# MIT-SPARK/Kimera-Semantics

Hardware: AMD Instinct MI355X
Metric: Mvoxel-updates/s + frames/s, 640×480 @5cm voxels, 1/2/4/8 MI355X (higher is better)
Workload: dtype f32; 1 GPU; bag-replay stand-in: 640x480 depth+label trajectory (room), 'fast' integrator, 5 cm voxels, 5 m rays, trunc 0.2 m, p=0.8; pipeline_frames=12, parallelism=frame-sharded x1, points_per_frame=305657, rays_per_frame=85307, updates_per_frame=502687

## Files before the change

kimera_semantics_amd/csrc/ks_hip.hip:

```cpp

#include <atomic>
#include <chrono>
#include <condition_variable>
#include <mutex>
#include <thread>
#include <cstring>
#include <string.h>

#include <dlfcn.h>
#include <hip/hip_runtime.h>
#include <hip/hip_ext.h>
#include <rccl/rccl.h>

#include <algorithm>
#include <iterator>
#include <cmath>
#include <cstdio>
#include <cstring>
#include <string>
#include <unordered_map>
#include <vector>

#include "../../include/ks_hip.h"
#include "ks_device_math.h"
// ... 880 lines not shown
                       (const uint32_t*)vres, c->d_eo_plain);
  return KS_OK;
}

int ensure_exact_slots(ks_ctx* c, size_t cap_marks, size_t cap_x) {
  if (!c->eo_device) return KS_OK;
  int rc;
  const int n_slots = c->cfg.pipeline_frames ? c->n_slots : 1;
  for (int i = 0; i < n_slots; ++i) {
    FrameSlot& S = c->slot[i];
    if (!S.d_eo_ctl) {
      if ((rc = S.d_eo_ctl.alloc(c, 1))) return rc;
      if ((rc = S.d_eo_tab.alloc(c, (size_t)1 << kSetBits))) return rc;
      HIPCHK(c, hipMemsetAsync(S.d_eo_tab, 0, sizeof(uint4) << kSetBits, c->stream));
      if ((rc = S.eo_committed.create(c, hipEventDisableTiming))) return rc;
    }
    if (S.eo_cap_marks < cap_marks) {
      S.eo_cap_marks = 0;
      for (int b = 0; b < 2; ++b) {
        if ((rc = S.d_eo_keys[b].alloc(c, cap_marks))) return rc;
        if ((rc = S.d_eo_vals[b].alloc(c, cap_marks))) return rc;
      }
      if ((rc = S.d_eo_sort_ws.alloc(c, ksrs::ws_words_dev(cap_marks, 3)))) return rc;
      if ((rc = S.d_eo_hitb.alloc(c, cap_marks))) return rc;
      if ((rc = S.d_eo_hseq.alloc(c, cap_marks))) return rc;
      if ((rc = S.d_eo_where.alloc(c, cap_marks))) return rc;
      if ((rc = S.d_eo_bits_a.alloc(c, cap_marks / 64 + 2))) return rc;
      if ((rc = S.d_eo_bits_b.alloc(c, cap_marks / 64 + 2))) return rc;
      S.eo_cap_marks = cap_marks;
    }
    if ((rc = S.d_eo_xnode.reserve(c, 2 * cap_x, 2 * cap_x))) return rc;
  }
  c->eo_cap_marks = cap_marks;
  c->eo_cap_x = cap_x;
  ++c->buffers_epoch;
  HIPCHK(c, hipStreamSynchronize(c->stream));
  return KS_OK;
}
int ensure_exact_points(ks_ctx* c, size_t cap) {
  if (!c->eo_device) return KS_OK;
  int rc;
  for (int i = 0; i < (c->cfg.pipeline_frames ? c->n_slots : 1); ++i) {
    FrameSlot& S = c->slot[i];
    for (DevBuf<uint32_t>* p : {&S.d_eo_cnt_b, &S.d_eo_ux, &S.d_eo_dirty, &S.d_eo_list[0], &S.d_eo_list[1], &S.d_eo_chg, &S.d_eo_consulted, &S.d_eo_lp})
      if ((rc = p->alloc(c, cap))) return rc;
    if ((rc = S.d_eo_bt.alloc(c, cap / kScanBlock + 2))) return rc;
// ... 78 lines not shown
    hipLaunchKernelGGL(k_eo2_scan, dim3(nb4k, nb), dim3(1024), 0, st, Bt);
    hipLaunchKernelGGL(k_eo2_emit<8>, dim3((uint32_t)((n + 31) / 32), nb), dim3(256), lds, st, Bt);
    HIPCHK(c, ksrs::sort_dev_batch<uint64_t>(Rs, (int)nb, S0.d_eo_sort_ws.size(), S0.eo_cap_marks, 44, 64, st));
    hipLaunchKernelGGL(k_eo2_bits, dim3(gm, nb), dim3(256), 0, st, Bt, 0u);
    hipLaunchKernelGGL(k_eo2_where, dim3(gm, nb), dim3(256), 0, st, Bt);
    enqueue_sweeps(c, Bt, nb, c->eo_sweeps, st);
    return KS_OK;
  } else {
    hipLaunchKernelGGL(k_eo2_scan, dim3(nb4k, nb), dim3(1024), 0, st, Bt);
    hipLaunchKernelGGL(k_eo2_emit<64>, dim3((uint32_t)((n + 255) / 256), nb), dim3(256), lds, st, Bt);
    HIPCHK(c, ksrs::sort_dev_batch<uint64_t>(Rs, (int)nb, S0.d_eo_sort_ws.size(), S0.eo_cap_marks, 44, 64, st));
    hipLaunchKernelGGL(k_eo2_hits, dim3(gm, nb), dim3(256), 0, st, Bt);
    hipLaunchKernelGGL(k_eo2_stop0, dim3(gn, nb), dim3(256), 0, st, Bt);
    hipLaunchKernelGGL(k_eo2_bits, dim3(gm, nb), dim3(256), 0, st, Bt, 1u);
  }
  const uint32_t gr = (uint32_t)std::min<size_t>((n + 3) / 4, 2048);
  for (int r = 1; r <= c->eo_bulk_rounds; ++r) {
    const uint32_t g = S0.wide ? gr : std::min(gr, r == 1 ? 2048u : r == 2 ? 1024u : r <= 4 ? 512u : 256u);
    hipLaunchKernelGGL(k_eo2_eval, dim3(g, nb), dim3(256), 0, st, Bt, (uint32_t)r);
    hipLaunchKernelGGL(k_eo2_propagate, dim3(g, nb), dim3(256), 0, st, Bt, (uint32_t)r);
  }
  return KS_OK;
}
void enqueue_exact_finish(ks_ctx* c, FrameSlot& S, hipStream_t st) {
  const EoView E = eo_view(c, S);
  hipLaunchKernelGGL(k_eo2_finish, dim3(1), dim3(kEoFinishThreads), 0, st, E, (uint32_t)c->eo_bulk_rounds + 1u, 1u);
  hipLaunchKernelGGL(k_eo2_commit, dim3(1024), dim3(256), 0, st, E);
}

template <typename Enqueue> hipGraphExec_t capture_graph(hipStream_t sm, Enqueue enqueue) {
  hipGraph_t g = nullptr;
  hipGraphExec_t out = nullptr;
  bool ok = hipStreamBeginCapture(sm, hipStreamCaptureModeRelaxed) == hipSuccess;
  if (ok) {
    const int rc = enqueue();
    ok = hipStreamEndCapture(sm, &g) == hipSuccess && g != nullptr && rc == KS_OK;
  }
  if (ok) ok = hipGraphInstantiate(&out, g, nullptr, nullptr, 0) == hipSuccess;
  if (g) (void)hipGraphDestroy(g);
  return ok ? out : nullptr;
}
struct BatchLaunch {
  ks_ctx* c;
  FrameSlot* const* slots;
  uint32_t nb;
  FrameSlot& S0;
  hipStream_t sm;
  const BatchView& V;
  size_t steps_max;
  uint64_t key;
// ... 3 lines not shown
    for (uint32_t k = 0; k < nb; ++k) Bt.v[k] = eo_view(c, *slots[k]);
    for (int chunk = 1;; ++chunk) {
      bool going = false;
      for (uint32_t k = 0; k < nb; ++k) {
        uint32_t w[2] = {0u, 0u};
        HIPCHK(c, hipMemcpyAsync(&w[0], &slots[k]->d_eo_ctl->sw_prev, sizeof(uint32_t), hipMemcpyDeviceToHost, sm));
        HIPCHK(c, hipMemcpyAsync(&w[1], &slots[k]->d_eo_ctl->fail, sizeof(uint32_t), hipMemcpyDeviceToHost, sm));
        HIPCHK(c, hipStreamSynchronize(sm));
        going = going || (w[0] != 0u && w[1] == 0u);
      }
      if (!going || chunk >= c->eo_sweep_chunks) break;
      enqueue_sweeps(c, Bt, nb, c->eo_sweeps, sm);
    }
    hipLaunchKernelGGL(k_eo2_sweep_done, dim3(nb), dim3(64), 0, sm, Bt);
    return KS_OK;
  }
  int exact_device() const {
    int rc;
    auto seed_and_rounds = [&] {
      enqueue_stage_b(c, V, nb, S0.wide, sm, steps_max, 1);
      return enqueue_exact_rounds(c, slots, nb, sm);
    };
    auto finish = [&] {
      for (uint32_t k = 0; k < nb; ++k) enqueue_exact_finish(c, *slots[k], sm);
      return KS_OK;
    };
    auto emission = [&] { return enqueue_stage_b(c, V, nb, S0.wide, sm, steps_max, 2), KS_OK; };
    bool graphs = c->use_graphs && !S0.wide;
    if (graphs && (G.key != key || !G.g1 || !G.g2 || !G.g3)) {
      std::lock_guard<std::mutex> cap(c->capture_mu);
      G.reset();
      if ((G.g1 = capture_graph(sm, seed_and_rounds)) && (G.g2 = capture_graph(sm, finish)) && (G.g3 = capture_graph(sm, emission))) {
        G.key = key;
      } else {
        (void)hipGetLastError();
        G.reset();
        c->use_graphs = graphs = false;
      }
    }
    if (graphs) HIPCHK(c, hipGraphLaunch(G.g1, sm));
    else if ((rc = seed_and_rounds()) || (S0.wide && (rc = sweeps_host_driven()))) return rc;
    if (c->eo_last_commit && c->eo_last_commit != S0.eo_committed) HIPCHK(c, hipStreamWaitEvent(sm, c->eo_last_commit, 0));
    if (graphs) HIPCHK(c, hipGraphLaunch(G.g2, sm));
    else finish();
    HIPCHK(c, hipEventRecord(S0.eo_committed, sm));
    c->eo_last_commit = S0.eo_committed;
    if (graphs) HIPCHK(c, hipGraphLaunch(G.g3, sm));
// ... 103 lines not shown
  F.clear_bit = (cfg.method == KS_METHOD_MERGED) ? (1u << pb) : 0u;
  F.seq_bits = pb + (cfg.method == KS_METHOD_MERGED ? 1u : 0u);
  F.inv_order = F.sorted_order ? c->d_inv_order : nullptr;
  std::memcpy(F.dynamic_labels, cfg.dynamic_labels, 32);
  F.early_out = c->uses_early_out;
}
void begin_prof_set(ks_ctx* c, FrameSlot& S, size_t n) {
  const int set = (int)(c->frame_no % kProfSets);
  resolve_prof(c, set);
  ProfSet& P = c->pset[set];
  P.used = true;
  P.complete = P.applied = false;
  P.stages = c->profiling == 1;
  P.apply = c->profiling == 1 || (c->frame_no % 4) == 0;
  P.n_points = n;
  P.n_pairs = 0;
  S.prof_set = set;
}
int stage_a_fast(ks_ctx* c, FrameSlot& S, const float* d_xyz, const uint8_t* d_rgba, const uint8_t* d_labels, size_t n) {
  const FrameParams& F = S.F;
  hipStream_t st = c->stream;
  const uint32_t nb1k = (uint32_t)((n + 1023) / 1024);
  hipLaunchKernelGGL(k_points_fast, dim3(nb1k), dim3(1024), 0, st, F, d_xyz, d_rgba, d_labels, c->d_color_lut,
                     S.d_rays, c->d_hash, c->d_skeys32, c->d_pvals, S.d_cnt, S.d_live, S.d_counters);
  stage_mark(c, S.prof_set, 1);
  uint32_t *sk = nullptr, *sv = nullptr;
  if (int rc = sort_pairs(c, c->d_skeys32.get(), c->d_skeys32b.get(), c->d_pvals.get(), c->d_pvals2.get(), n, kSetBits + 1, &sk, &sv)) return rc;
  stage_mark(c, S.prof_set, 2);
  hipLaunchKernelGGL(k_dedup, dim3(nb1k), dim3(1024), 0, st, F, sk, sv, c->d_hash, c->d_start_set, S.d_ray_list, S.d_rays, S.d_cnt, S.d_live, S.d_counters);
  if (c->uses_early_out && n > 0) {
    const uint32_t n_gen = (uint32_t)((n + F.chains - 1) / F.chains);
    uint32_t n_ph = 0;
    while (n_ph < c->seed_phases.size() && c->seed_phases[n_ph].g0 < n_gen) ++n_ph;
    HIPCHK(c, hipMemsetAsync(S.d_seed_n, 0, c->seed_phases.size() * sizeof(uint32_t), st));
    hipLaunchKernelGGL(k_seed_list, dim3((F.chains + 63u) / 64u, n_ph), dim3(64 * kSeedSegs), 0, st, F, (const SeedPhase*)c->d_seed_phases,
                       (const uint8_t*)S.d_live, S.d_seed_gen, S.d_seed_items, S.d_seed_n, S.d_counters);
  }
  hipLaunchKernelGGL(k_dedup_commit, dim3(nb1k), dim3(1024), 0, st, F, sk, sv, c->d_hash, c->d_start_set, S.d_counters);
  return KS_OK;
}
void enqueue_bundle_order(ks_ctx* c, hipStream_t st, size_t n, const uint64_t* sk, const uint32_t* sv) {
  const uint32_t capb = (uint32_t)((c->cap_points + kBoBlock - 1) / kBoBlock);
  const size_t lds_f = (2 * c->cap_points / kBoBlock + 3) * sizeof(uint32_t), lds_e = ((size_t)capb + 2) * sizeof(uint32_t);
  hipLaunchKernelGGL(k_bo_scan_flags, dim3((uint32_t)((2 * n + kBoBlock - 1) / kBoBlock)), dim3(kBoBlock), 0, st, (uint32_t)n, c->bo);
  hipLaunchKernelGGL(k_bo_init, dim3((uint32_t)((n + kBoBlock - 1) / kBoBlock)), dim3(kBoBlock), lds_f, st, (uint32_t)n, sk, sv, c->bo);
  const uint32_t nbb = (uint32_t)((n + kBoBlock - 1) / kBoBlock);
  int e_small = 0;
  while (e_small < c->bo_epochs && c->bo_sched.b[e_small] <= kBoSmallBuckets) ++e_small;
  if (e_small > 0) hipLaunchKernelGGL(k_bo_small, dim3(2), dim3(kBoBlock), 0, st, c->bo, e_small);
  const size_t nh_floor = c->bo_hint_fixed ? (e_small > 0 ? (size_t)c->bo_sched.t[e_small - 1] + 1 : 1) : 2 * (size_t)kBoSmallBuckets;
  const size_t nh = std::min<size_t>(n, std::max<size_t>(c->bo_hint.load(std::memory_order_relaxed), nh_floor));
  int e_last = -1;
  for (int e = e_small; e <= c->bo_epochs; ++e) {
    if (e > 0 && c->bo_sched.t[e - 1] >= nh) break;
    hipLaunchKernelGGL(k_bo_link, dim3(nbb, 2), dim3(kBoBlock), lds_e, st, c->bo, e, (e == e_small && e_small > 0) ? 1 : 0);
    if (e < c->bo_epochs && c->bo_sched.t[e] < nh)
      hipLaunchKernelGGL(k_bo_walk, dim3(nbb, 2), dim3(kBoBlock), 0, st, c->bo, e);
// ... 2330 lines not shown
}

int ks_debug_radix_sort_batch(ks_ctx* c, uint64_t* keys, uint32_t* vals, const uint64_t* counts, int nb, size_t cap, unsigned begin_bit,
                              unsigned end_bit) {
  if (!c || !keys || !vals || !counts || nb < 1 || nb > ksrs::kRsBatch || cap == 0 || cap > 0xffffffffull || begin_bit >= end_bit || end_bit > 64)
    return KS_ERR_INVALID_ARG;
  const int passes = (int)((end_bit - begin_bit + 7) / 8);
  const size_t ws_words = ksrs::ws_words_dev(cap, passes);
  DevBuf<uint64_t> ka[ksrs::kRsBatch], kb[ksrs::kRsBatch];
  DevBuf<uint32_t> va[ksrs::kRsBatch], vb[ksrs::kRsBatch], ws[ksrs::kRsBatch];
  DevBuf<unsigned long long> d_counts;
  int rc;
  if ((rc = d_counts.alloc(c, (size_t)nb))) return rc;
  static_assert(sizeof(unsigned long long) == sizeof(uint64_t), "counts are copied as they are");
  HIPCHK(c, hipMemcpy(d_counts, counts, (size_t)nb * sizeof(uint64_t), hipMemcpyHostToDevice));
  ksrs::DevBatch<uint64_t> B{};
  for (int y = 0; y < nb; ++y) {
    if ((rc = ka[y].alloc(c, cap)) || (rc = kb[y].alloc(c, cap)) || (rc = va[y].alloc(c, cap)) || (rc = vb[y].alloc(c, cap)) || (rc = ws[y].alloc(c, ws_words)))
      return rc;
    HIPCHK(c, hipMemcpy(ka[y], keys + (size_t)y * cap, cap * sizeof(uint64_t), hipMemcpyHostToDevice));
    HIPCHK(c, hipMemcpy(va[y], vals + (size_t)y * cap, cap * sizeof(uint32_t), hipMemcpyHostToDevice));
    HIPCHK(c, hipMemsetAsync(kb[y], 0xA5, cap * sizeof(uint64_t), c->stream));
    HIPCHK(c, hipMemsetAsync(vb[y], 0xA5, cap * sizeof(uint32_t), c->stream));
    B.keys_a[y] = ka[y];
    B.keys_b[y] = kb[y];
    B.vals_a[y] = va[y];
    B.vals_b[y] = vb[y];
    B.n_dev[y] = d_counts.get() + y;
    B.ws[y] = ws[y];
  }
  const hipError_t e = ksrs::sort_dev_batch<uint64_t>(B, nb, ws_words, cap, begin_bit, end_bit, c->stream);
  if (e == hipErrorInvalidValue) return KS_ERR_INVALID_ARG;
  HIPCHK(c, e);
  HIPCHK(c, hipStreamSynchronize(c->stream));
  const bool in_b = (passes & 1) != 0;
  for (int y = 0; y < nb; ++y) {
    HIPCHK(c, hipMemcpy(keys + (size_t)y * cap, in_b ? kb[y].get() : ka[y].get(), cap * sizeof(uint64_t), hipMemcpyDeviceToHost));
    HIPCHK(c, hipMemcpy(vals + (size_t)y * cap, in_b ? vb[y].get() : va[y].get(), cap * sizeof(uint32_t), hipMemcpyDeviceToHost));
  }
  return KS_OK;
}

int ks_get_tile_keys(ks_ctx* c, uint64_t* out, size_t cap, size_t* n) {
  if (!c || !n) return KS_ERR_INVALID_ARG;
  if (int rc = quiesce(c)) return rc;
  HIPCHK(c, hipStreamSynchronize(c->stream));
// ... 1049 lines not shown
```

kimera_semantics_amd/csrc/ks_k_exact.h:

```cpp
#pragma once
#include "ks_k_march.h"

namespace ksk {

struct EoState {
  unsigned long long n_marks;
  unsigned long long n_marks_next;
  uint32_t changed;
  uint32_t pad[3];
};

struct EoBuf {
  const uint64_t* keys;
  const uint32_t* vals;
  uint2* range;
  uint64_t* plain;
};
constexpr uint64_t kEoLow44 = (1ull << 44) - 1ull;

__device__ __forceinline__ uint32_t eo_visited(uint32_t cv) { return (cv & ~kCntBroke) + ((cv & kCntBroke) ? 1u : 0u); }

__global__ void __launch_bounds__(256) k_eo_total(const FrameParams* __restrict__ Fp, const uint32_t* __restrict__ cnt,
                                                  EoState* __restrict__ st) {
  const uint32_t n = Fp->n;
// ... 983 lines not shown
  const EoView& E = Bt.v[blockIdx.y];
  EoCtl* ctl = E.ctl;
  if (ctl->fail) return;
  const uint32_t n = ctl->n_in[round];
  const uint32_t* list = E.list[round & 1u];
  const uint32_t wave = threadIdx.x >> 6, w0 = blockIdx.x * 4u + wave, nw = gridDim.x * 4u;
  if (w0 >= n) return;
  const FrameParams F = *E.F;
  for (uint32_t i = w0; i < n; i += nw) eo2_eval_ray(E, F, list[i], s_w[wave], &ctl->n_chg[round]);
}
__global__ void __launch_bounds__(256) k_eo2_propagate(EoBatch Bt, uint32_t round) {
  __shared__ EoWaveLds s_w[4];
  const EoView& E = Bt.v[blockIdx.y];
  EoCtl* ctl = E.ctl;
  if (ctl->fail) return;
  const uint32_t n = ctl->n_chg[round];
  const uint32_t wave = threadIdx.x >> 6, w0 = blockIdx.x * 4u + wave, nw = gridDim.x * 4u;
  if (blockIdx.x == 0 && threadIdx.x == 0 && n) ctl->rounds = round + 1u;
  if (w0 >= n) return;
  const FrameParams F = *E.F;
  for (uint32_t i = w0; i < n; i += nw) eo2_propagate_ray(E, F, E.chg[i], s_w[wave], E.list[(round + 1u) & 1u], &ctl->n_in[round + 1u]);
}

constexpr uint32_t kEoFinishThreads = 1024;
__global__ void __launch_bounds__(kEoFinishThreads) k_eo2_finish(EoView E, uint32_t first_round, uint32_t chained) {
  __shared__ EoWaveLds s_w[kEoFinishThreads / 64];
  __shared__ uint32_t s_n, s_stop;
  EoCtl* ctl = E.ctl;
  const uint32_t wave = threadIdx.x >> 6, nw = kEoFinishThreads / 64;
  const FrameParams F = *E.F;
  uint32_t cur = first_round & 1u;
  if (threadIdx.x == 0) {
    if (chained && eo2_ld(E.committed) != F.eo_frame) atomicOr(&ctl->fail, kEoFailChain);
    ctl->fin_in[cur] = ctl->n_in[first_round];
    ctl->fin_in[cur ^ 1u] = 0u;
    ctl->fin_chg = 0u;
    s_stop = ctl->fail;
  }
  __syncthreads();
  if (s_stop) {
    if (threadIdx.x == 0) atomicOr(&E.C->err, kErrExact);
    return;
  }
  if (chained) {
    __shared__ uint32_t s_redo;
    if (threadIdx.x == 0) {
      const unsigned long long actual = E.plain[(uint32_t)(F.observed_offset & kSetMask)];
      s_redo = actual != ctl->assumed0 ? 1u : 0u;
      ctl->assumed0 = actual;
    }
    __syncthreads();
    if (s_redo) {
      const uint32_t nc = eo2_ld(&ctl->n_consulted);
      for (uint32_t i = threadIdx.x; i < nc; i += kEoFinishThreads) eo2_mark_dirty(E, eo2_ld(&E.consulted[i]), 0u, E.list[cur], &ctl->fin_in[cur]);
    }
    __syncthreads();
  }
  for (uint32_t it = 0;; ++it) {
    if (threadIdx.x == 0) {
      s_n = eo2_ld(&ctl->fin_in[cur]);
      s_stop = eo2_ld(&ctl->fail) | ((it >= kEoFinishRounds || s_n > kEoFinishRays) ? kEoFailRounds : 0u);
      if (s_n && !s_stop) ctl->rounds += 1u;
    }
    __syncthreads();
    const uint32_t n = s_n;
    if (n == 0u || s_stop) break;
    for (uint32_t i = wave; i < n; i += nw) eo2_eval_ray(E, F, eo2_ld(&E.list[cur][i]), s_w[wave], &ctl->fin_chg);
    __syncthreads();
    if (threadIdx.x == 0) {
      s_n = eo2_ld(&ctl->fin_chg);
      ctl->fin_in[cur] = 0u;
    }
    __syncthreads();
    const uint32_t nc = s_n;
    for (uint32_t i = wave; i < nc; i += nw) eo2_propagate_ray(E, F, eo2_ld(&E.chg[i]), s_w[wave], E.list[cur ^ 1u], &ctl->fin_in[cur ^ 1u]);
    __syncthreads();
    if (threadIdx.x == 0) ctl->fin_chg = 0u;
    cur ^= 1u;
  }
  if (threadIdx.x == 0 && s_stop) {
    atomicOr(&ctl->fail, s_stop);
    atomicOr(&E.C->err, kErrExact);
  }
}

__global__ void __launch_bounds__(256) k_eo2_commit(EoView E) {
  const bool ok = E.ctl->fail == 0u;
  for (uint32_t slot = blockIdx.x * 256u + threadIdx.x; slot < (1u << kSetBits); slot += gridDim.x * 256u) {
    const uint4 e = E.tab[slot];
    if (e.x == e.y && e.z == 0u) continue;
    E.tab[slot] = make_uint4(0u, 0u, 0u, 0u);
    if (!ok) continue;
    bool found = false;
    uint64_t best = 0;
    uint32_t hash = 0;
    if (e.y > e.x) {
      const long long j = eo2_prev_set(E.bits_a, e.y);
      if (j >= (long long)e.x) {
        found = true;
        best = E.keys[j] & kEoLow44;
        hash = E.vals[j];
      }
    }
    for (uint32_t xi = e.z; xi != 0u;) {
      const unsigned long long k = E.xnode[2u * xi], hn = E.xnode[2u * xi + 1u];
      if (((uint32_t)k & 0x3fffffu) < eo_visited(E.cnt_a[(uint32_t)(k >> 22)]) && (!found || k > best)) {
        found = true;
        best = k;
        hash = (uint32_t)hn;
      }
      xi = (uint32_t)(hn >> 32);
    }
    if (found) E.plain[slot] = (uint64_t)hash;
  }
  if (ok && blockIdx.x == 0 && threadIdx.x == 0) *E.committed = E.F->eo_frame + 1u;
}

__global__ void __launch_bounds__(64) k_eo2_begin(EoBatch Bt) {
  const EoView& E = Bt.v[blockIdx.x];
  EoCtl* ctl = E.ctl;
  uint32_t* w = (uint32_t*)ctl;
  for (uint32_t i = threadIdx.x; i < sizeof(EoCtl) / 4u; i += 64) w[i] = 0u;
  __syncthreads();
  if (threadIdx.x == 0) {
    ctl->n_x = 1u;
    ctl->sw_prev = 1u;
    ctl->sw_full = 1u;
    ctl->assumed0 = E.plain[(uint32_t)(E.F->observed_offset & kSetMask)];
  }
}

}
```

kimera_semantics_amd/csrc/ks_k_rays.h:

```cpp
#pragma once
#include "ks_types.h"
#include "ks_k_bundle_order.h"

namespace ksk {
__global__ void __launch_bounds__(1024) k_points_fast(FrameParams F, const float* __restrict__ xyz,
                                                      const uint8_t* __restrict__ rgba,
                                                      const uint8_t* __restrict__ labels,
                                                      const uint8_t* __restrict__ color_lut,
                                                      RayDesc* __restrict__ rays, uint32_t* __restrict__ hash_out,
                                                      uint32_t* __restrict__ keys, uint32_t* __restrict__ vals,
                                                      uint32_t* __restrict__ cnt, uint8_t* __restrict__ live,
                                                      Counters* C) {
  const uint32_t idx = blockIdx.x * blockDim.x + threadIdx.x;
  bool counted = false;
  if (idx < F.n) {
    cnt[idx] = 0u;
    live[idx] = 0;
    uint32_t key = kInvalidSlot;
    const f3 pc = {xyz[3 * idx], xyz[3 * idx + 1], xyz[3 * idx + 2]};
    uint32_t color = 0;
    if (rgba) color = ((const uint32_t*)rgba)[idx];
    uint32_t label;
    if (labels) label = labels[idx];
    else label = color_lut ? color_lut[color & 0xffffffu] : 0u;
    if (label >= (uint32_t)kNumLabels) {
      atomicOr(&C->err, kErrLabel);
    } else {
      int valid = point_validity(pc, F.min_ray, F.max_ray, F.allow_clear != 0, F.freespace != 0);
      for (int i = 0; i < F.n_dynamic; ++i)
        if (F.dynamic_labels[i] == label) valid = 0;
      if (valid) {
        const f3 pg = transform_point(F.T, pc);
        const float gx = grid_coord(pg.x, F.start_inv), gy = grid_coord(pg.y, F.start_inv),
                    gz = grid_coord(pg.z, F.start_inv);
        const float lim = 2.0f * (float)kCoordBias;
// ... 494 lines not shown
```

kimera_semantics_amd/csrc/ks_radix_sort.h:

```cpp
#pragma once
#include <hip/hip_runtime.h>
#include <stdint.h>
#include <algorithm>
#include <stdlib.h>

#include "ks_owned.h"

namespace ksrs {

constexpr int kMaxPasses = 8;
constexpr int kMaxBins = 2048;
constexpr size_t kHistBlocks = 2048;
constexpr uint32_t kFlagLocal = 1u << 30, kFlagPrefix = 2u << 30, kCountMask = (1u << 30) - 1u;

template <typename K>
__device__ __forceinline__ uint32_t digit_of(K key, int shift, uint32_t mask) {
  return (uint32_t)(key >> shift) & mask;
}
inline uint32_t last_digit_mask(unsigned begin_bit, unsigned end_bit, int rb) {
  const unsigned rem = (end_bit - begin_bit) - ((end_bit - begin_bit + rb - 1) / rb - 1) * rb;
  return (1u << rem) - 1u;
}

template <int RB>
__device__ __forceinline__ unsigned long long match_digit(uint32_t d, unsigned long long active) {
  unsigned long long peers = active;
#pragma unroll
  for (int b = 0; b < RB; ++b) {
    const bool bit = (d >> b) & 1u;
    const unsigned long long bal = __ballot(bit);
    peers &= bit ? bal : ~bal;
  }
  return peers;
}

// ... 39 lines not shown
  __syncthreads();
  for (int i = tid; i < passes * kBins; i += 256) {
    const uint32_t c = s_hist[i];
    if (c) atomicAdd(&hist[(i / kBins) * kMaxBins + (i % kBins)], c);
  }
}
template <typename K, int RB>
__global__ void __launch_bounds__(256) k_rs_hist(const K* __restrict__ keys, uint32_t n, int passes, int begin_bit, uint32_t last_mask,
                                                 uint32_t* __restrict__ hist, uint32_t* __restrict__ zero_ptr,
                                                 uint32_t zero_words) {
  extern __shared__ uint32_t s_hist[];
  rs_hist_body<K, RB>(keys, n, passes, begin_bit, last_mask, hist, zero_ptr, zero_words, nullptr, s_hist);
}
constexpr int kRsBatch = 8;
template <typename K>
struct DevBatch {
  K* keys_a[kRsBatch];
  K* keys_b[kRsBatch];
  uint32_t* vals_a[kRsBatch];
  uint32_t* vals_b[kRsBatch];
  const unsigned long long* n_dev[kRsBatch];
  uint32_t* ws[kRsBatch];
};
template <typename K, int RB>
__global__ void __launch_bounds__(256) k_rs_hist_b(DevBatch<K> B, uint32_t cap, int passes, int begin_bit, uint32_t last_mask) {
  extern __shared__ uint32_t s_hist[];
  rs_hist_body<K, RB>(B.keys_a[blockIdx.y], cap, passes, begin_bit, last_mask, B.ws[blockIdx.y], nullptr, 0u, B.n_dev[blockIdx.y], s_hist);
}

template <typename K, bool HAS_VALUES, int THREADS, int ITEMS, int RB, bool REORDER = false>
__device__ __forceinline__ void rs_pass_body(const K* __restrict__ keys_in, K* __restrict__ keys_out,
                                             const uint32_t* __restrict__ vals_in,
                                             uint32_t* __restrict__ vals_out, uint32_t n, int shift, uint32_t mask,
                                             const uint32_t* __restrict__ bin_hist,
                                             uint32_t* __restrict__ status, uint32_t* __restrict__ ticket,
                                             const unsigned long long* __restrict__ n_dev) {
  constexpr int kBins = 1 << RB;
  constexpr int kChunks = kBins / 64;
  constexpr int kWaves = THREADS / 64;
  constexpr int kTile = THREADS * ITEMS;
  if (n_dev) n = (uint32_t)(*n_dev < (unsigned long long)n ? *n_dev : (unsigned long long)n);
  __shared__ uint32_t s_cnt[kWaves][kBins];
  __shared__ uint32_t s_off[kBins];
  __shared__ uint32_t s_chunk[kChunks];
  __shared__ uint32_t s_tile;
  __shared__ K s_keys[REORDER ? kTile : 1];
  __shared__ uint32_t s_loc[REORDER ? kBins : 1];
  static_assert(!REORDER || (!HAS_VALUES && kBins <= THREADS), "reorder variant: keys only");
  const uint32_t tid = threadIdx.x, lane = tid & 63u, wave = tid >> 6;
  if (tid == 0) s_tile = ticket ? atomicAdd(ticket, 1u) : blockIdx.x;
// ... 120 lines not shown
    return;
  }
#pragma unroll
  for (int i = 0; i < ITEMS; ++i) {
    const uint32_t idx = wbase + i * 64 + lane;
    if (idx < n) {
      const uint32_t d = rd[i] >> 20;
      const uint32_t pos = s_off[d] + s_cnt[wave][d] + (rd[i] & 0xfffffu);
      keys_out[pos] = key[i];
      if (HAS_VALUES) vals_out[pos] = vals_in[idx];
    }
  }
}

template <typename K, bool HAS_VALUES, int THREADS, int ITEMS, int RB, bool REORDER = false>
__global__ void __launch_bounds__(THREADS) k_rs_pass(const K* __restrict__ keys_in, K* __restrict__ keys_out,
                                                     const uint32_t* __restrict__ vals_in,
                                                     uint32_t* __restrict__ vals_out, uint32_t n, int shift, uint32_t mask,
                                                     const uint32_t* __restrict__ bin_hist,
                                                     uint32_t* __restrict__ status, uint32_t* __restrict__ ticket) {
  rs_pass_body<K, HAS_VALUES, THREADS, ITEMS, RB, REORDER>(keys_in, keys_out, vals_in, vals_out, n, shift, mask, bin_hist, status, ticket, nullptr);
}
template <typename K, int THREADS, int ITEMS, int RB>
__global__ void __launch_bounds__(THREADS) k_rs_pass_b(DevBatch<K> B, uint32_t cap, int begin_bit, int p, uint32_t tiles, uint32_t mask) {
  const uint32_t y = blockIdx.y;
  uint32_t* ws = B.ws[y];
  const bool odd = (p & 1) != 0;
  rs_pass_body<K, true, THREADS, ITEMS, RB, false>(odd ? B.keys_b[y] : B.keys_a[y], odd ? B.keys_a[y] : B.keys_b[y], odd ? B.vals_b[y] : B.vals_a[y],
                                                   odd ? B.vals_a[y] : B.vals_b[y], cap, begin_bit + p * RB, mask, ws + (size_t)p * kMaxBins,
                                                   ws + ((size_t)kMaxPasses * kMaxBins + kMaxPasses) + (size_t)p * tiles * (1 << RB),
                                                   ws + (size_t)kMaxPasses * kMaxBins + p, B.n_dev[y]);
}

struct Workspace {
  DevBuf<uint32_t> d_ws;
  size_t words = 0;
  int cur = 0;
  size_t dirty[2] = {0, 0};
};
constexpr size_t kHeadWords = (size_t)kMaxPasses * kMaxBins + kMaxPasses;

inline hipError_t ensure(Workspace& w, size_t words, hipStream_t stream) {
  if (words <= w.words) return hipSuccess;
  w.words = 0;
  const size_t cap = ((words + words / 4) + 3) & ~(size_t)3;
  hipError_t e = w.d_ws.try_alloc(2 * cap);
  if (e != hipSuccess) return e;
  e = hipMemsetAsync(w.d_ws, 0, 2 * cap * sizeof(uint32_t), stream);
  if (e != hipSuccess) return e;
  w.words = cap;
  w.cur = 0;
  w.dirty[0] = w.dirty[1] = 0;
  return hipSuccess;
}

template <typename K, bool HAS_VALUES, int THREADS, int ITEMS, int RB, bool REORDER = false>
inline void launch_passes(Workspace& w, K*& kin, K*& kout, uint32_t*& vin, uint32_t*& vout, size_t n, int passes,
                          uint32_t tiles, unsigned begin_bit, uint32_t last_mask, hipStream_t stream) {
  constexpr int kBins = 1 << RB;
  uint32_t* base = w.d_ws + (size_t)w.cur * w.words;
  uint32_t* hist = base;
  uint32_t* tickets = base + (size_t)kMaxPasses * kMaxBins;
  uint32_t* status = base + kHeadWords;
// ... 22 lines not shown
  const int h = w.cur ^ 1;
  hipLaunchKernelGGL((k_rs_hist<K, RB>), dim3((uint32_t)std::min<size_t>((n + 2047) / 2048, kHistBlocks)), dim3(256),
                     (size_t)passes * kBins * sizeof(uint32_t), stream, keys_a, (uint32_t)n, passes, (int)begin_bit, last_mask,
                     w.d_ws + (size_t)h * w.words, w.d_ws + (size_t)(h ^ 1) * w.words,
                     (uint32_t)((w.dirty[h ^ 1] + 3) & ~(size_t)3));
  w.dirty[h ^ 1] = 0;
  w.dirty[h] = words;
  w.cur = h;
  K* kin = keys_a;
  K* kout = keys_b;
  uint32_t* vin = vals_a;
  uint32_t* vout = vals_b;
  if (tile == 2048) launch_passes<K, HAS_VALUES, 256, 8, RB>(w, kin, kout, vin, vout, n, passes, tiles, begin_bit, last_mask, stream);
  else if (tile == 8192 && reorder) {
    if constexpr (!HAS_VALUES) launch_passes<K, false, 512, 16, RB, true>(w, kin, kout, vin, vout, n, passes, tiles, begin_bit, last_mask, stream);
  } else if (tile == 8192) launch_passes<K, HAS_VALUES, 512, 16, RB>(w, kin, kout, vin, vout, n, passes, tiles, begin_bit, last_mask, stream);
  else launch_passes<K, HAS_VALUES, 512, 32, RB>(w, kin, kout, vin, vout, n, passes, tiles, begin_bit, last_mask, stream);
  *keys_result = kin;
  if (vals_result) *vals_result = vin;
  return hipGetLastError();
}

inline size_t dev_tile(size_t cap) { return cap <= (1u << 20) ? 2048 : cap <= (1u << 24) ? 8192 : 16384; }
inline size_t ws_words_dev(size_t cap, int passes) { return kHeadWords + (size_t)passes * ((cap + dev_tile(cap) - 1) / dev_tile(cap)) * 256; }

template <typename K>
inline hipError_t sort_dev_batch(const DevBatch<K>& B, int nb, size_t ws_words, size_t cap, unsigned begin_bit, unsigned end_bit, hipStream_t stream) {
  constexpr int RB = 8;
  constexpr int kBins = 1 << RB;
  const int passes = (int)((end_bit - begin_bit + RB - 1) / RB);
  const uint32_t last_mask = last_digit_mask(begin_bit, end_bit, RB);
  const size_t tile = dev_tile(cap);
  const uint32_t tiles = (uint32_t)((cap + tile - 1) / tile);
  if (kHeadWords + (size_t)passes * tiles * kBins > ws_words || nb < 1 || nb > kRsBatch) return hipErrorInvalidValue;
  for (int y = 0; y < nb; ++y) {
    hipError_t e = hipMemsetAsync(B.ws[y], 0, (kHeadWords + (size_t)passes * tiles * kBins) * sizeof(uint32_t), stream);
    if (e != hipSuccess) return e;
  }
  hipLaunchKernelGGL((k_rs_hist_b<K, RB>), dim3((uint32_t)std::min<size_t>((cap + 2047) / 2048, kHistBlocks), (uint32_t)nb), dim3(256),
                     (size_t)passes * kBins * sizeof(uint32_t), stream, B, (uint32_t)cap, passes, (int)begin_bit, last_mask);
  for (int p = 0; p < passes; ++p) {
    const uint32_t mask = p == passes - 1 ? last_mask : (uint32_t)(kBins - 1);
    if (tile == 2048) hipLaunchKernelGGL((k_rs_pass_b<K, 256, 8, RB>), dim3(tiles, (uint32_t)nb), dim3(256), 0, stream, B, (uint32_t)cap, (int)begin_bit, p, tiles, mask);
    else if (tile == 8192) hipLaunchKernelGGL((k_rs_pass_b<K, 512, 16, RB>), dim3(tiles, (uint32_t)nb), dim3(512), 0, stream, B, (uint32_t)cap, (int)begin_bit, p, tiles, mask);
    else hipLaunchKernelGGL((k_rs_pass_b<K, 512, 32, RB>), dim3(tiles, (uint32_t)nb), dim3(512), 0, stream, B, (uint32_t)cap, (int)begin_bit, p, tiles, mask);
  }
  return hipGetLastError();
}

template <typename K, bool HAS_VALUES>
inline hipError_t sort(Workspace& w, K* keys_a, K* keys_b, uint32_t* vals_a, uint32_t* vals_b, size_t n,
                       unsigned end_bit, hipStream_t stream, K** keys_result, uint32_t** vals_result,
                       unsigned begin_bit = 0) {
  *keys_result = keys_a;
  if (vals_result) *vals_result = vals_a;
  if (end_bit > sizeof(K) * 8) end_bit = (unsigned)(sizeof(K) * 8);
  if (n == 0 || end_bit <= begin_bit) return hipSuccess;
  return sort_rb<K, HAS_VALUES, 8>(w, keys_a, keys_b, vals_a, vals_b, n, begin_bit, end_bit, stream, keys_result, vals_result);
}

}
```

Before: 1013 Mvoxel-updates/s.

## Batch exact-finish/commit kernels and fold per-sort memsets into kernels

Replaces per-frame finish and commit launches with single batched kernels that process all frames in a batch sequentially inside one block, resolving the cross-frame slot dependency in-kernel. Removes the per-call workspace memsets in the batched radix sort by double-buffering the workspace and having the histogram kernel clear the previous half. Also folds the seed counter memset into the points kernel. The goal is fewer launches and memset nodes per frame, at the cost of a serialized one-block finish across frames and more complex workspace state.

```diff
diff --git a/kimera_semantics_amd/csrc/ks_hip.hip b/kimera_semantics_amd/csrc/ks_hip.hip
--- a/kimera_semantics_amd/csrc/ks_hip.hip
+++ b/kimera_semantics_amd/csrc/ks_hip.hip
@@ -926,6 +926,7 @@
         if ((rc = S.d_eo_vals[b].alloc(c, cap_marks))) return rc;
       }
       if ((rc = S.d_eo_sort_ws.alloc(c, ksrs::ws_words_dev(cap_marks, 3)))) return rc;
+      HIPCHK(c, ksrs::init_dev_ws(S.d_eo_sort_ws, S.d_eo_sort_ws.size(), c->stream));
       if ((rc = S.d_eo_hitb.alloc(c, cap_marks))) return rc;
       if ((rc = S.d_eo_hseq.alloc(c, cap_marks))) return rc;
       if ((rc = S.d_eo_where.alloc(c, cap_marks))) return rc;
@@ -1050,10 +1051,11 @@
   }
   return KS_OK;
 }
-void enqueue_exact_finish(ks_ctx* c, FrameSlot& S, hipStream_t st) {
-  const EoView E = eo_view(c, S);
-  hipLaunchKernelGGL(k_eo2_finish, dim3(1), dim3(kEoFinishThreads), 0, st, E, (uint32_t)c->eo_bulk_rounds + 1u, 1u);
-  hipLaunchKernelGGL(k_eo2_commit, dim3(1024), dim3(256), 0, st, E);
+void enqueue_exact_finish(ks_ctx* c, FrameSlot* const* slots, uint32_t nb, hipStream_t st) {
+  EoBatch Bt{};
+  for (uint32_t k = 0; k < nb; ++k) Bt.v[k] = eo_view(c, *slots[k]);
+  hipLaunchKernelGGL(k_eo2_finish_batch, dim3(1), dim3(kEoFinishThreads), 0, st, Bt, nb, (uint32_t)c->eo_bulk_rounds + 1u);
+  hipLaunchKernelGGL(k_eo2_commit_batch, dim3(1024), dim3(256), 0, st, Bt, nb);
 }
 
 template <typename Enqueue> hipGraphExec_t capture_graph(hipStream_t sm, Enqueue enqueue) {
@@ -1103,7 +1105,7 @@
       return enqueue_exact_rounds(c, slots, nb, sm);
     };
     auto finish = [&] {
-      for (uint32_t k = 0; k < nb; ++k) enqueue_exact_finish(c, *slots[k], sm);
+      enqueue_exact_finish(c, slots, nb, sm);
       return KS_OK;
     };
     auto emission = [&] { return enqueue_stage_b(c, V, nb, S0.wide, sm, steps_max, 2), KS_OK; };
@@ -1253,7 +1255,8 @@
   hipStream_t st = c->stream;
   const uint32_t nb1k = (uint32_t)((n + 1023) / 1024);
   hipLaunchKernelGGL(k_points_fast, dim3(nb1k), dim3(1024), 0, st, F, d_xyz, d_rgba, d_labels, c->d_color_lut,
-                     S.d_rays, c->d_hash, c->d_skeys32, c->d_pvals, S.d_cnt, S.d_live, S.d_counters);
+                     S.d_rays, c->d_hash, c->d_skeys32, c->d_pvals, S.d_cnt, S.d_live, S.d_counters,
+                     c->uses_early_out ? S.d_seed_n.get() : nullptr, (uint32_t)c->seed_phases.size());
   stage_mark(c, S.prof_set, 1);
   uint32_t *sk = nullptr, *sv = nullptr;
   if (int rc = sort_pairs(c, c->d_skeys32.get(), c->d_skeys32b.get(), c->d_pvals.get(), c->d_pvals2.get(), n, kSetBits + 1, &sk, &sv)) return rc;
@@ -1263,7 +1266,6 @@
     const uint32_t n_gen = (uint32_t)((n + F.chains - 1) / F.chains);
     uint32_t n_ph = 0;
     while (n_ph < c->seed_phases.size() && c->seed_phases[n_ph].g0 < n_gen) ++n_ph;
-    HIPCHK(c, hipMemsetAsync(S.d_seed_n, 0, c->seed_phases.size() * sizeof(uint32_t), st));
     hipLaunchKernelGGL(k_seed_list, dim3((F.chains + 63u) / 64u, n_ph), dim3(64 * kSeedSegs), 0, st, F, (const SeedPhase*)c->d_seed_phases,
                        (const uint8_t*)S.d_live, S.d_seed_gen, S.d_seed_items, S.d_seed_n, S.d_counters);
   }
@@ -3640,6 +3642,7 @@
     HIPCHK(c, hipMemcpy(va[y], vals + (size_t)y * cap, cap * sizeof(uint32_t), hipMemcpyHostToDevice));
     HIPCHK(c, hipMemsetAsync(kb[y], 0xA5, cap * sizeof(uint64_t), c->stream));
     HIPCHK(c, hipMemsetAsync(vb[y], 0xA5, cap * sizeof(uint32_t), c->stream));
+    HIPCHK(c, ksrs::init_dev_ws(ws[y], ws_words, c->stream));
     B.keys_a[y] = ka[y];
     B.keys_b[y] = kb[y];
     B.vals_a[y] = va[y];
diff --git a/kimera_semantics_amd/csrc/ks_k_exact.h b/kimera_semantics_amd/csrc/ks_k_exact.h
--- a/kimera_semantics_amd/csrc/ks_k_exact.h
+++ b/kimera_semantics_amd/csrc/ks_k_exact.h
@@ -1029,30 +1029,66 @@
   for (uint32_t i = w0; i < n; i += nw) eo2_propagate_ray(E, F, E.chg[i], s_w[wave], E.list[(round + 1u) & 1u], &ctl->n_in[round + 1u]);
 }
 
+template <bool LIVE>
+__device__ __forceinline__ bool eo2_slot_final(const EoView& E, const uint4 e, uint32_t& hash) {
+  bool found = false;
+  uint64_t best = 0;
+  if (e.y > e.x) {
+    const long long j = LIVE ? eo2_prev_set_live(E.bits_a, e.y) : eo2_prev_set(E.bits_a, e.y);
+    if (j >= (long long)e.x) {
+      found = true;
+      best = E.keys[j] & kEoLow44;
+      hash = E.vals[j];
+    }
+  }
+  for (uint32_t xi = e.z; xi != 0u;) {
+    const unsigned long long k = LIVE ? eo2_ld64(&E.xnode[2u * xi]) : E.xnode[2u * xi];
+    const unsigned long long hn = LIVE ? eo2_ld64(&E.xnode[2u * xi + 1u]) : E.xnode[2u * xi + 1u];
+    const uint32_t len = LIVE ? eo2_ld(&E.cnt_a[(uint32_t)(k >> 22)]) : E.cnt_a[(uint32_t)(k >> 22)];
+    if (((uint32_t)k & 0x3fffffu) < eo_visited(len) && (!found || k > best)) {
+      found = true;
+      best = k;
+      hash = (uint32_t)hn;
+    }
+    xi = (uint32_t)(hn >> 32);
+  }
+  return found;
+}
+
 constexpr uint32_t kEoFinishThreads = 1024;
-__global__ void __launch_bounds__(kEoFinishThreads) k_eo2_finish(EoView E, uint32_t first_round, uint32_t chained) {
+__global__ void __launch_bounds__(kEoFinishThreads) k_eo2_finish_batch(EoBatch Bt, uint32_t nb, uint32_t first_round) {
   __shared__ EoWaveLds s_w[kEoFinishThreads / 64];
-  __shared__ uint32_t s_n, s_stop;
-  EoCtl* ctl = E.ctl;
+  __shared__ uint32_t s_n, s_stop, s_redo;
   const uint32_t wave = threadIdx.x >> 6, nw = kEoFinishThreads / 64;
-  const FrameParams F = *E.F;
-  uint32_t cur = first_round & 1u;
-  if (threadIdx.x == 0) {
-    if (chained && eo2_ld(E.committed) != F.eo_frame) atomicOr(&ctl->fail, kEoFailChain);
-    ctl->fin_in[cur] = ctl->n_in[first_round];
-    ctl->fin_in[cur ^ 1u] = 0u;
-    ctl->fin_chg = 0u;
-    s_stop = ctl->fail;
-  }
-  __syncthreads();
-  if (s_stop) {
-    if (threadIdx.x == 0) atomicOr(&E.C->err, kErrExact);
-    return;
-  }
-  if (chained) {
-    __shared__ uint32_t s_redo;
+  for (uint32_t f = 0; f < nb; ++f) {
+    const EoView& E = Bt.v[f];
+    EoCtl* ctl = E.ctl;
+    const FrameParams F = *E.F;
+    uint32_t cur = first_round & 1u;
+    __syncthreads();
     if (threadIdx.x == 0) {
-      const unsigned long long actual = E.plain[(uint32_t)(F.observed_offset & kSetMask)];
+      const bool broken = f == 0u ? eo2_ld(E.committed) != F.eo_frame : eo2_ld(&Bt.v[f - 1u].ctl->fail) != 0u;
+      if (broken) atomicOr(&ctl->fail, kEoFailChain);
+      ctl->fin_in[cur] = ctl->n_in[first_round];
+      ctl->fin_in[cur ^ 1u] = 0u;
+      ctl->fin_chg = 0u;
+      s_stop = ctl->fail;
+    }
+    __syncthreads();
+    if (s_stop) {
+      if (threadIdx.x == 0) atomicOr(&E.C->err, kErrExact);
+      continue;
+    }
+    if (threadIdx.x == 0) {
+      const uint32_t slot0 = (uint32_t)(F.observed_offset & kSetMask);
+      unsigned long long actual = E.plain[slot0];
+      for (uint32_t g = 0; g < f; ++g) {
+        const EoView& P = Bt.v[g];
+        uint4 e = P.tab[slot0];
+        e.z = eo2_ld(&P.tab[slot0].z);
+        uint32_t hash = 0;
+        if (eo2_slot_final<true>(P, e, hash)) actual = (unsigned long long)hash;
+      }
       s_redo = actual != ctl->assumed0 ? 1u : 0u;
       ctl->assumed0 = actual;
     }
@@ -1062,65 +1098,55 @@
       for (uint32_t i = threadIdx.x; i < nc; i += kEoFinishThreads) eo2_mark_dirty(E, eo2_ld(&E.consulted[i]), 0u, E.list[cur], &ctl->fin_in[cur]);
     }
     __syncthreads();
-  }
-  for (uint32_t it = 0;; ++it) {
-    if (threadIdx.x == 0) {
-      s_n = eo2_ld(&ctl->fin_in[cur]);
-      s_stop = eo2_ld(&ctl->fail) | ((it >= kEoFinishRounds || s_n > kEoFinishRays) ? kEoFailRounds : 0u);
-      if (s_n && !s_stop) ctl->rounds += 1u;
-    }
-    __syncthreads();
-    const uint32_t n = s_n;
-    if (n == 0u || s_stop) break;
-    for (uint32_t i = wave; i < n; i += nw) eo2_eval_ray(E, F, eo2_ld(&E.list[cur][i]), s_w[wave], &ctl->fin_chg);
-    __syncthreads();
-    if (threadIdx.x == 0) {
-      s_n = eo2_ld(&ctl->fin_chg);
-      ctl->fin_in[cur] = 0u;
-    }
-    __syncthreads();
-    const uint32_t nc = s_n;
-    for (uint32_t i = wave; i < nc; i += nw) eo2_propagate_ray(E, F, eo2_ld(&E.chg[i]), s_w[wave], E.list[cur ^ 1u], &ctl->fin_in[cur ^ 1u]);
-    __syncthreads();
-    if (threadIdx.x == 0) ctl->fin_chg = 0u;
-    cur ^= 1u;
-  }
-  if (threadIdx.x == 0 && s_stop) {
-    atomicOr(&ctl->fail, s_stop);
-    atomicOr(&E.C->err, kErrExact);
-  }
-}
-
-__global__ void __launch_bounds__(256) k_eo2_commit(EoView E) {
-  const bool ok = E.ctl->fail == 0u;
+    for (uint32_t it = 0;; ++it) {
+      if (threadIdx.x == 0) {
+        s_n = eo2_ld(&ctl->fin_in[cur]);
+        s_stop = eo2_ld(&ctl->fail) | ((it >= kEoFinishRounds || s_n > kEoFinishRays) ? kEoFailRounds : 0u);
+        if (s_n && !s_stop) ctl->rounds += 1u;
+      }
+      __syncthreads();
+      const uint32_t n = s_n;
+      if (n == 0u || s_stop) break;
+      for (uint32_t i = wave; i < n; i += nw) eo2_eval_ray(E, F, eo2_ld(&E.list[cur][i]), s_w[wave], &ctl->fin_chg);
+      __syncthreads();
+      if (threadIdx.x == 0) {
+        s_n = eo2_ld(&ctl->fin_chg);
+        ctl->fin_in[cur] = 0u;
+      }
+      __syncthreads();
+      const uint32_t nc = s_n;
+      for (uint32_t i = wave; i < nc; i += nw) eo2_propagate_ray(E, F, eo2_ld(&E.chg[i]), s_w[wave], E.list[cur ^ 1u], &ctl->fin_in[cur ^ 1u]);
+      __syncthreads();
+      if (threadIdx.x == 0) ctl->fin_chg = 0u;
+      cur ^= 1u;
+    }
+    if (threadIdx.x == 0 && s_stop) {
+      atomicOr(&ctl->fail, s_stop);
+      atomicOr(&E.C->err, kErrExact);
+    }
+  }
+}
+
+__global__ void __launch_bounds__(256) k_eo2_commit_batch(EoBatch Bt, uint32_t nb) {
+  uint32_t n_ok = 0;
+  while (n_ok < nb && Bt.v[n_ok].ctl->fail == 0u) ++n_ok;
+  uint64_t* plain = Bt.v[0].plain;
   for (uint32_t slot = blockIdx.x * 256u + threadIdx.x; slot < (1u << kSetBits); slot += gridDim.x * 256u) {
-    const uint4 e = E.tab[slot];
-    if (e.x == e.y && e.z == 0u) continue;
-    E.tab[slot] = make_uint4(0u, 0u, 0u, 0u);
-    if (!ok) continue;
+    uint4 e[kBatchMax];
+#pragma unroll
+    for (uint32_t f = 0; f < (uint32_t)kBatchMax; ++f)
+      if (f < nb) e[f] = Bt.v[f].tab[slot];
     bool found = false;
-    uint64_t best = 0;
     uint32_t hash = 0;
-    if (e.y > e.x) {
-      const long long j = eo2_prev_set(E.bits_a, e.y);
-      if (j >= (long long)e.x) {
-        found = true;
-        best = E.keys[j] & kEoLow44;
-        hash = E.vals[j];
-      }
-    }
-    for (uint32_t xi = e.z; xi != 0u;) {
-      const unsigned long long k = E.xnode[2u * xi], hn = E.xnode[2u * xi + 1u];
-      if (((uint32_t)k & 0x3fffffu) < eo_visited(E.cnt_a[(uint32_t)(k >> 22)]) && (!found || k > best)) {
-        found = true;
-        best = k;
-        hash = (uint32_t)hn;
-      }
-      xi = (uint32_t)(hn >> 32);
-    }
-    if (found) E.plain[slot] = (uint64_t)hash;
-  }
-  if (ok && blockIdx.x == 0 && threadIdx.x == 0) *E.committed = E.F->eo_frame + 1u;
+#pragma unroll
+    for (uint32_t f = 0; f < (uint32_t)kBatchMax; ++f) {
+      if (f >= nb || (e[f].x == e[f].y && e[f].z == 0u)) continue;
+      Bt.v[f].tab[slot] = make_uint4(0u, 0u, 0u, 0u);
+      if (f < n_ok && eo2_slot_final<false>(Bt.v[f], e[f], hash)) found = true;
+    }
+    if (found) plain[slot] = (uint64_t)hash;
+  }
+  if (n_ok && blockIdx.x == 0 && threadIdx.x == 0) *Bt.v[0].committed = Bt.v[n_ok - 1u].F->eo_frame + 1u;
 }
 
 __global__ void __launch_bounds__(64) k_eo2_begin(EoBatch Bt) {
diff --git a/kimera_semantics_amd/csrc/ks_k_rays.h b/kimera_semantics_amd/csrc/ks_k_rays.h
--- a/kimera_semantics_amd/csrc/ks_k_rays.h
+++ b/kimera_semantics_amd/csrc/ks_k_rays.h
@@ -10,7 +10,9 @@
                                                       RayDesc* __restrict__ rays, uint32_t* __restrict__ hash_out,
                                                       uint32_t* __restrict__ keys, uint32_t* __restrict__ vals,
                                                       uint32_t* __restrict__ cnt, uint8_t* __restrict__ live,
-                                                      Counters* C) {
+                                                      Counters* C, uint32_t* __restrict__ seed_n, uint32_t n_seed) {
+  if (blockIdx.x == 0 && seed_n)
+    for (uint32_t i = threadIdx.x; i < n_seed; i += blockDim.x) seed_n[i] = 0u;
   const uint32_t idx = blockIdx.x * blockDim.x + threadIdx.x;
   bool counted = false;
   if (idx < F.n) {
diff --git a/kimera_semantics_amd/csrc/ks_radix_sort.h b/kimera_semantics_amd/csrc/ks_radix_sort.h
--- a/kimera_semantics_amd/csrc/ks_radix_sort.h
+++ b/kimera_semantics_amd/csrc/ks_radix_sort.h
@@ -11,6 +11,7 @@
 constexpr int kMaxPasses = 8;
 constexpr int kMaxBins = 2048;
 constexpr size_t kHistBlocks = 2048;
+constexpr size_t kHeadWords = (size_t)kMaxPasses * kMaxBins + kMaxPasses;
 constexpr uint32_t kFlagLocal = 1u << 30, kFlagPrefix = 2u << 30, kCountMask = (1u << 30) - 1u;
 
 template <typename K>
@@ -96,10 +97,28 @@
   const unsigned long long* n_dev[kRsBatch];
   uint32_t* ws[kRsBatch];
 };
+constexpr size_t kWsHeader = 4;
 template <typename K, int RB>
-__global__ void __launch_bounds__(256) k_rs_hist_b(DevBatch<K> B, uint32_t cap, int passes, int begin_bit, uint32_t last_mask) {
+__global__ void __launch_bounds__(256) k_rs_hist_b(DevBatch<K> B, uint32_t cap, int passes, int begin_bit, uint32_t last_mask, uint32_t half_words,
+                                                   uint32_t tiles, uint32_t tile) {
   extern __shared__ uint32_t s_hist[];
-  rs_hist_body<K, RB>(B.keys_a[blockIdx.y], cap, passes, begin_bit, last_mask, B.ws[blockIdx.y], nullptr, 0u, B.n_dev[blockIdx.y], s_hist);
+  uint32_t* ws = B.ws[blockIdx.y];
+  const uint32_t prev = ws[0] & 1u, cur = prev ^ 1u;
+  const unsigned long long nd = *B.n_dev[blockIdx.y];
+  const uint32_t n = (uint32_t)(nd < (unsigned long long)cap ? nd : (unsigned long long)cap);
+  const uint32_t n_prev = ws[2u + prev];
+  if (blockIdx.x == 0 && threadIdx.x == 0) {
+    ws[1] = cur;
+    ws[2u + cur] = n;
+  }
+  uint4* z = (uint4*)(ws + kWsHeader + (size_t)prev * half_words);
+  const uint32_t head4 = (uint32_t)(kHeadWords / 4), row4 = ((n_prev + tile - 1u) / tile) * ((1u << RB) / 4u);
+  for (uint32_t i = blockIdx.x * 256u + threadIdx.x; i < head4 + (uint32_t)passes * row4; i += gridDim.x * 256u) {
+    const uint32_t j = i - head4;
+    z[i < head4 ? i : head4 + (j / row4) * (tiles * ((1u << RB) / 4u)) + j % row4] = make_uint4(0u, 0u, 0u, 0u);
+  }
+  rs_hist_body<K, RB>(B.keys_a[blockIdx.y], cap, passes, begin_bit, last_mask, ws + kWsHeader + (size_t)cur * half_words, nullptr, 0u,
+                      B.n_dev[blockIdx.y], s_hist);
 }
 
 template <typename K, bool HAS_VALUES, int THREADS, int ITEMS, int RB, bool REORDER = false>
@@ -266,9 +285,11 @@
   rs_pass_body<K, HAS_VALUES, THREADS, ITEMS, RB, REORDER>(keys_in, keys_out, vals_in, vals_out, n, shift, mask, bin_hist, status, ticket, nullptr);
 }
 template <typename K, int THREADS, int ITEMS, int RB>
-__global__ void __launch_bounds__(THREADS) k_rs_pass_b(DevBatch<K> B, uint32_t cap, int begin_bit, int p, uint32_t tiles, uint32_t mask) {
+__global__ void __launch_bounds__(THREADS) k_rs_pass_b(DevBatch<K> B, uint32_t cap, int begin_bit, int p, uint32_t tiles, uint32_t mask, uint32_t half_words) {
   const uint32_t y = blockIdx.y;
-  uint32_t* ws = B.ws[y];
+  const uint32_t cur = B.ws[y][1] & 1u;
+  if (p == 0 && blockIdx.x == 0 && threadIdx.x == 0) B.ws[y][0] = cur;
+  uint32_t* ws = B.ws[y] + kWsHeader + (size_t)cur * half_words;
   const bool odd = (p & 1) != 0;
   rs_pass_body<K, true, THREADS, ITEMS, RB, false>(odd ? B.keys_b[y] : B.keys_a[y], odd ? B.keys_a[y] : B.keys_b[y], odd ? B.vals_b[y] : B.vals_a[y],
                                                    odd ? B.vals_a[y] : B.vals_b[y], cap, begin_bit + p * RB, mask, ws + (size_t)p * kMaxBins,
@@ -282,7 +303,6 @@
   int cur = 0;
   size_t dirty[2] = {0, 0};
 };
-constexpr size_t kHeadWords = (size_t)kMaxPasses * kMaxBins + kMaxPasses;
 
 inline hipError_t ensure(Workspace& w, size_t words, hipStream_t stream) {
   if (words <= w.words) return hipSuccess;
@@ -351,7 +371,9 @@
 }
 
 inline size_t dev_tile(size_t cap) { return cap <= (1u << 20) ? 2048 : cap <= (1u << 24) ? 8192 : 16384; }
-inline size_t ws_words_dev(size_t cap, int passes) { return kHeadWords + (size_t)passes * ((cap + dev_tile(cap) - 1) / dev_tile(cap)) * 256; }
+inline size_t ws_half_words(size_t cap, int passes) { return kHeadWords + (size_t)passes * ((cap + dev_tile(cap) - 1) / dev_tile(cap)) * 256; }
+inline size_t ws_words_dev(size_t cap, int passes) { return kWsHeader + 2 * ws_half_words(cap, passes); }
+inline hipError_t init_dev_ws(uint32_t* ws, size_t ws_words, hipStream_t stream) { return hipMemsetAsync(ws, 0, ws_words * sizeof(uint32_t), stream); }
 
 template <typename K>
 inline hipError_t sort_dev_batch(const DevBatch<K>& B, int nb, size_t ws_words, size_t cap, unsigned begin_bit, unsigned end_bit, hipStream_t stream) {
@@ -361,18 +383,16 @@
   const uint32_t last_mask = last_digit_mask(begin_bit, end_bit, RB);
   const size_t tile = dev_tile(cap);
   const uint32_t tiles = (uint32_t)((cap + tile - 1) / tile);
-  if (kHeadWords + (size_t)passes * tiles * kBins > ws_words || nb < 1 || nb > kRsBatch) return hipErrorInvalidValue;
-  for (int y = 0; y < nb; ++y) {
-    hipError_t e = hipMemsetAsync(B.ws[y], 0, (kHeadWords + (size_t)passes * tiles * kBins) * sizeof(uint32_t), stream);
-    if (e != hipSuccess) return e;
-  }
+  const size_t half = ws_half_words(cap, passes);
+  if (ws_words_dev(cap, passes) > ws_words || half > 0xffffffffull || nb < 1 || nb > kRsBatch) return hipErrorInvalidValue;
   hipLaunchKernelGGL((k_rs_hist_b<K, RB>), dim3((uint32_t)std::min<size_t>((cap + 2047) / 2048, kHistBlocks), (uint32_t)nb), dim3(256),
-                     (size_t)passes * kBins * sizeof(uint32_t), stream, B, (uint32_t)cap, passes, (int)begin_bit, last_mask);
+                     (size_t)passes * kBins * sizeof(uint32_t), stream, B, (uint32_t)cap, passes, (int)begin_bit, last_mask, (uint32_t)half, tiles,
+                     (uint32_t)tile);
   for (int p = 0; p < passes; ++p) {
     const uint32_t mask = p == passes - 1 ? last_mask : (uint32_t)(kBins - 1);
-    if (tile == 2048) hipLaunchKernelGGL((k_rs_pass_b<K, 256, 8, RB>), dim3(tiles, (uint32_t)nb), dim3(256), 0, stream, B, (uint32_t)cap, (int)begin_bit, p, tiles, mask);
-    else if (tile == 8192) hipLaunchKernelGGL((k_rs_pass_b<K, 512, 16, RB>), dim3(tiles, (uint32_t)nb), dim3(512), 0, stream, B, (uint32_t)cap, (int)begin_bit, p, tiles, mask);
-    else hipLaunchKernelGGL((k_rs_pass_b<K, 512, 32, RB>), dim3(tiles, (uint32_t)nb), dim3(512), 0, stream, B, (uint32_t)cap, (int)begin_bit, p, tiles, mask);
+    if (tile == 2048) hipLaunchKernelGGL((k_rs_pass_b<K, 256, 8, RB>), dim3(tiles, (uint32_t)nb), dim3(256), 0, stream, B, (uint32_t)cap, (int)begin_bit, p, tiles, mask, (uint32_t)half);
+    else if (tile == 8192) hipLaunchKernelGGL((k_rs_pass_b<K, 512, 16, RB>), dim3(tiles, (uint32_t)nb), dim3(512), 0, stream, B, (uint32_t)cap, (int)begin_bit, p, tiles, mask, (uint32_t)half);
+    else hipLaunchKernelGGL((k_rs_pass_b<K, 512, 32, RB>), dim3(tiles, (uint32_t)nb), dim3(512), 0, stream, B, (uint32_t)cap, (int)begin_bit, p, tiles, mask, (uint32_t)half);
   }
   return hipGetLastError();
 }
```

Measured after the change: 1021 Mvoxel-updates/s, median of 6. Within noise of the previous version (+0.8%).
